# dherrera1911/sqfa

Measured on AMD Instinct MI355X. Metric: SPD pairwise-distance loss+grad evals/sec, higher is better.
Workload: dtype f32; 1 GPU; c3: C=1000 classes, n_dim=784, n_filters=16, smsqfa (m=16), 499500 unordered pairs per eval, inputs resident in HBM; parallelism=pair-tile shard over 1 GPU(s) + 1 all-reduce of [loss,flags,grad] per eval

## Files before the change

### include/sqfa_hip.h

```cpp
#ifndef SQFA_HIP_H
#define SQFA_HIP_H

#include <stddef.h>

#ifdef __cplusplus
extern "C" {
#endif

#define SQFA_F32 0
#define SQFA_F64 1

#define SQFA_OK                 0
#define SQFA_ERR_BAD_ARGUMENT  -1
#define SQFA_ERR_UNSUPPORTED_M -2
#define SQFA_ERR_WORKSPACE     -3
#define SQFA_ERR_LAUNCH        -4

int sqfa_hip_version(void);
const char *sqfa_hip_arch(void);
int sqfa_hip_max_dim(void);

const char *sqfa_hip_last_error(void);

int sqfa_airm_tiling(int nA, int nB, int m, int dtype,
                     int *tile_i, int *tile_j, int *n_tiles_i, int *n_tiles_j, int *padded_m);

size_t sqfa_airm_workspace_bytes(int nA, int nB, int m, int dtype);
size_t sqfa_airm_workspace_bytes_sharded(int nA, int nB, int m, int dtype, int shard_count, int geometry_policy);

typedef struct sqfa_airm_options {
  int geometry_policy;
  int class_factor_policy;
  unsigned long long *sweep_counter;
  int mean_metric_policy;
} sqfa_airm_options;

int sqfa_airm_pairwise(const void *A, int nA, const void *B, int nB, int m, int dtype,
                       double scale, double eps, int sqrt_mode,
                       const void *pair_weights, double uniform_weight,
                       int shard_index, int shard_count,
                       void *loss_out, void *gradA_out, void *gradB_out,
                       void *dist_out, void *eig_out, int *nonfinite_out,
                       void *workspace, size_t workspace_bytes, void *stream);
int sqfa_airm_pairwise_opt(const void *A, int nA, const void *B, int nB, int m, int dtype,
                           double scale, double eps, int sqrt_mode,
                           const void *pair_weights, double uniform_weight,
                           int shard_index, int shard_count,
                           void *loss_out, void *gradA_out, void *gradB_out,
                           void *dist_out, void *eig_out, int *nonfinite_out,
                           void *workspace, size_t workspace_bytes, void *stream,
                           const sqfa_airm_options *options);

size_t sqfa_bw_workspace_bytes(int nA, int nB, int m, int dtype);
size_t sqfa_bw_workspace_bytes_sharded(int nA, int nB, int m, int dtype, int shard_count, int geometry_policy);
int sqfa_bw_pairwise(const void *A, int nA, const void *B, int nB, int m, int dtype,
                     double eps, int sqrt_mode,
                     const void *pair_weights, double uniform_weight,
                     int shard_index, int shard_count,
                     void *loss_out, void *gradA_out, void *gradB_out,
                     void *dist_out, int *nonfinite_out,
                     void *workspace, size_t workspace_bytes, void *stream,
                     const sqfa_airm_options *options);

int sqfa_airm_eigenvalues_backward(const void *A, int nA, const void *B, int nB, int m, int dtype,
                                   const void *eig_weights, void *gradA_out, void *gradB_out,
                                   void *workspace, size_t workspace_bytes, void *stream,
                                   const sqfa_airm_options *options);

int sqfa_project_scatters(const void *F, int K, int D, const void *Psi, int C, int dtype, void *T_out,
                          void *stream);

size_t sqfa_packed_scatter_elems(int D);
int sqfa_pack_scatters(const void *Psi, int C, int D, int dtype, void *packed_out, void *stream);
int sqfa_project_scatters_packed(const void *F, int K, int D, const void *packed, int C, int dtype, void *T_out,
                                 void *stream);

int sqfa_feature_scatters(const void *F, int K, int D, const void *T, int C, int dtype, void *S_out, void *stream);
int sqfa_feature_scatters_backward(const void *G, const void *T, int C, int D, int K, int dtype, int n_groups,
                                   void *partial_out, void *stream);

int sqfa_feature_scatters_ex(const void *F, int K, int D, const void *T, int C, int dtype, double noise,
                             const void *means_f, void *S_out, void *stream);
int sqfa_feature_scatters_backward_ex(const void *G, int ldg, const void *T, int C, int D, int K, int dtype,
                                      int n_groups, int g_symmetric, void *partial_out, void *stream);
int sqfa_embed_backward_means(const void *gE, const void *means_f, int C, int K, int dtype, void *gm_out, void *stream);
int sqfa_sphere_forward(const void *X, int K, int D, int dtype, void *F_out, void *norms_out, void *stream);
int sqfa_sphere_backward(const void *X, const void *norms, int K, int D, int dtype, const void *partials, int n_groups,
                         const void *extra, const void *gloss, void *grad_out, void *stream);

int sqfa_lbfgs_max_history(void);
size_t sqfa_lbfgs_work_elems(int h, int n);
int sqfa_lbfgs_push(void *S, void *Y, void *SY, int h, int n, int slot, const void *s, const void *y, void *work,
                    int dtype, void *stream);
int sqfa_lbfgs_step_stats(const void *g, const void *g_prev, const void *d, double t, int n, void *y_out, void *s_out,
                          void *scalars_out, void *work, int dtype, void *stream);
int sqfa_lbfgs_direction(const void *S, const void *Y, const void *SY, int h, int n, const int *slots, int k,
                         const void *g, const void *H_diag, void *d_out, void *work, int dtype, void *stream);

int sqfa_gauss_pair_terms(const void *muA, const void *covA, int nA, const void *muB, const void *covB, int nB,
                          int m, int dtype, const void *gQ, const void *gLD, void *Q_out, void *LD_out,
                          void *gmuA_out, void *gcovA_out, void *stream);

#define SQFA_GAUSS_BHATTACHARYYA  0
#define SQFA_GAUSS_HELLINGER      1
// ... 26 lines not shown
```

### sqfa_amd/_lib.py

```python
import ctypes
import os

_HERE = os.path.dirname(os.path.abspath(__file__))
LIB_PATH = os.environ.get("SQFA_HIP_LIBRARY") or os.path.join(_HERE, "lib", "libsqfa_hip.so")

SQFA_F32, SQFA_F64 = 0, 1
SQFA_GAUSS_BHATTACHARYYA, SQFA_GAUSS_HELLINGER, SQFA_GAUSS_MAHALANOBIS_SQ, SQFA_GAUSS_MAHALANOBIS = 0, 1, 2, 3
SQFA_OK = 0
STATUS_TEXT = {
    -1: "bad argument",
    -2: "matrix size not supported by the native kernels",
    -3: "workspace too small",
    -4: "HIP launch failed",
}

class AirmOptions(ctypes.Structure):
    _fields_ = [("geometry_policy", ctypes.c_int), ("class_factor_policy", ctypes.c_int),
                ("sweep_counter", ctypes.c_void_p), ("mean_metric_policy", ctypes.c_int)]


_PAIRWISE_ARGS = [ctypes.c_void_p, ctypes.c_int, ctypes.c_void_p, ctypes.c_int, ctypes.c_int, ctypes.c_int,
                  ctypes.c_double, ctypes.c_double, ctypes.c_int,
                  ctypes.c_void_p, ctypes.c_double,
                  ctypes.c_int, ctypes.c_int,
                  ctypes.c_void_p, ctypes.c_void_p, ctypes.c_void_p,
                  ctypes.c_void_p, ctypes.c_void_p, ctypes.c_void_p,
                  ctypes.c_void_p, ctypes.c_size_t, ctypes.c_void_p]

_c_int_p = ctypes.POINTER(ctypes.c_int)
PROTOTYPES = {
    "sqfa_hip_version": (ctypes.c_int, []),
    "sqfa_hip_arch": (ctypes.c_char_p, []),
    "sqfa_hip_max_dim": (ctypes.c_int, []),
    "sqfa_hip_last_error": (ctypes.c_char_p, []),
    "sqfa_airm_tiling": (ctypes.c_int, [ctypes.c_int] * 4 + [_c_int_p] * 5),
    "sqfa_airm_workspace_bytes": (ctypes.c_size_t, [ctypes.c_int] * 4),
    "sqfa_airm_workspace_bytes_sharded": (ctypes.c_size_t, [ctypes.c_int] * 6),
    "sqfa_airm_pairwise": (ctypes.c_int, list(_PAIRWISE_ARGS)),
    "sqfa_airm_pairwise_opt": (ctypes.c_int, list(_PAIRWISE_ARGS) + [ctypes.POINTER(AirmOptions)]),
    "sqfa_bw_workspace_bytes": (ctypes.c_size_t, [ctypes.c_int] * 4),
    "sqfa_bw_workspace_bytes_sharded": (ctypes.c_size_t, [ctypes.c_int] * 6),
    "sqfa_bw_pairwise": (
        ctypes.c_int,
        [ctypes.c_void_p, ctypes.c_int, ctypes.c_void_p, ctypes.c_int, ctypes.c_int, ctypes.c_int,
         ctypes.c_double, ctypes.c_int, ctypes.c_void_p, ctypes.c_double, ctypes.c_int, ctypes.c_int,
         ctypes.c_void_p, ctypes.c_void_p, ctypes.c_void_p, ctypes.c_void_p, ctypes.c_void_p,
         ctypes.c_void_p, ctypes.c_size_t, ctypes.c_void_p, ctypes.POINTER(AirmOptions)],
    ),
    "sqfa_airm_eigenvalues_backward": (
        ctypes.c_int,
        [ctypes.c_void_p, ctypes.c_int, ctypes.c_void_p, ctypes.c_int, ctypes.c_int, ctypes.c_int,
         ctypes.c_void_p, ctypes.c_void_p, ctypes.c_void_p, ctypes.c_void_p, ctypes.c_size_t, ctypes.c_void_p,
         ctypes.POINTER(AirmOptions)],
    ),
    "sqfa_gauss_pair_terms": (
        ctypes.c_int,
        [ctypes.c_void_p, ctypes.c_void_p, ctypes.c_int, ctypes.c_void_p, ctypes.c_void_p, ctypes.c_int,
         ctypes.c_int, ctypes.c_int, ctypes.c_void_p, ctypes.c_void_p, ctypes.c_void_p, ctypes.c_void_p,
         ctypes.c_void_p, ctypes.c_void_p, ctypes.c_void_p],
    ),
    "sqfa_gauss_pairwise_workspace_bytes": (ctypes.c_size_t, [ctypes.c_int] * 3),
    "sqfa_gauss_pairwise_loss": (
        ctypes.c_int,
        [ctypes.c_void_p, ctypes.c_void_p, ctypes.c_int, ctypes.c_int, ctypes.c_int, ctypes.c_int,
         ctypes.c_double, ctypes.c_double, ctypes.c_void_p, ctypes.c_void_p, ctypes.c_void_p, ctypes.c_void_p,
         ctypes.c_void_p, ctypes.c_void_p, ctypes.c_size_t, ctypes.c_void_p],
    ),
    "sqfa_project_scatters": (
        ctypes.c_int,
        [ctypes.c_void_p, ctypes.c_int, ctypes.c_int, ctypes.c_void_p, ctypes.c_int, ctypes.c_int,
         ctypes.c_void_p, ctypes.c_void_p],
    ),
    "sqfa_packed_scatter_elems": (ctypes.c_size_t, [ctypes.c_int]),
    "sqfa_pack_scatters": (
        ctypes.c_int,
        [ctypes.c_void_p, ctypes.c_int, ctypes.c_int, ctypes.c_int, ctypes.c_void_p, ctypes.c_void_p],
    ),
    "sqfa_project_scatters_packed": (
        ctypes.c_int,
        [ctypes.c_void_p, ctypes.c_int, ctypes.c_int, ctypes.c_void_p, ctypes.c_int, ctypes.c_int,
         ctypes.c_void_p, ctypes.c_void_p],
    ),
    "sqfa_feature_scatters": (
        ctypes.c_int,
        [ctypes.c_void_p, ctypes.c_int, ctypes.c_int, ctypes.c_void_p, ctypes.c_int, ctypes.c_int,
         ctypes.c_void_p, ctypes.c_void_p],
    ),
    "sqfa_feature_scatters_backward": (
        ctypes.c_int,
        [ctypes.c_void_p, ctypes.c_void_p, ctypes.c_int, ctypes.c_int, ctypes.c_int, ctypes.c_int, ctypes.c_int,
         ctypes.c_void_p, ctypes.c_void_p],
    ),
# ... 89 lines not shown
```

### sqfa_amd/csrc/pair_inst.hip

```cpp
#include <type_traits>

#include "configs.hpp"
#include "pair_kernel.hpp"

#define SQFA_CAT_(a, b, c) a##b##_##c
#define SQFA_CAT(a, b, c) SQFA_CAT_(a, b, c)

#if defined(SQFA_RS) && SQFA_RS != 0
#include "pair_kernel_2d.hpp"
#define SQFA_ROW2D_MATCHES(T, MR, GC, CPL, TJ, WV, RS) \
  || (std::is_same<T, SQFA_T>::value && MR == SQFA_MR && GC == SQFA_G && CPL == SQFA_CPL && TJ == SQFA_TJ && WV == SQFA_WAVES && RS == SQFA_RS)
static_assert(false SQFA_CONFIGS2D_F32(SQFA_ROW2D_MATCHES) SQFA_CONFIGS2D_F64(SQFA_ROW2D_MATCHES),
              "Makefile CONFIGS2D and configs.hpp disagree");
namespace sqfa {
hipError_t SQFA_CAT(launch_pair2d_, SQFA_TAG, SQFA_MR)(const PairParams& p, hipStream_t stream) {
  return launch_pair_tiles_2d<PairCfg2D<SQFA_T, SQFA_MR, SQFA_G, SQFA_CPL, SQFA_TJ, SQFA_WAVES, SQFA_RS>>(p, stream);
}
hipError_t SQFA_CAT(launch_pair2d_bw_, SQFA_TAG, SQFA_MR)(const PairParams& p, hipStream_t stream) {
  return launch_pair_tiles_2d_bw<PairCfg2D<SQFA_T, SQFA_MR, SQFA_G, SQFA_CPL, SQFA_TJ, SQFA_WAVES, SQFA_RS>>(p, stream);
}
hipError_t SQFA_CAT(launch_factor2d_, SQFA_TAG, SQFA_MR)(const PairParams& p, hipStream_t stream) {
  return launch_class_factors<PairCfg2D<SQFA_T, SQFA_MR, SQFA_G, SQFA_CPL, SQFA_TJ, SQFA_WAVES, SQFA_RS>>(p, stream);
}
hipError_t SQFA_CAT(launch_classeig2d_, SQFA_TAG, SQFA_MR)(const void* LT, int n, int m, double* U, double* lam, hipStream_t stream) {
  return launch_class_eig<PairCfg2D<SQFA_T, SQFA_MR, SQFA_G, SQFA_CPL, SQFA_TJ, SQFA_WAVES, SQFA_RS>>(LT, n, m, U, lam, stream);
}
}
#else
#define SQFA_ROW_MATCHES(T, MR, G, CPL, TJ, WV) \
  || (std::is_same<T, SQFA_T>::value && MR == SQFA_MR && G == SQFA_G && CPL == SQFA_CPL && TJ == SQFA_TJ && WV == SQFA_WAVES)
static_assert(false SQFA_CONFIGS_F32(SQFA_ROW_MATCHES) SQFA_CONFIGS_F64(SQFA_ROW_MATCHES) SQFA_CONFIGS_F32_SMALL(SQFA_ROW_MATCHES)
              SQFA_CONFIGS_F64_SMALL(SQFA_ROW_MATCHES),
              "Makefile CONFIGS / CONFIGS_SMALL and configs.hpp disagree");
namespace sqfa {
hipError_t SQFA_CAT(launch_pair_, SQFA_TAG, SQFA_MR)(const PairParams& p, hipStream_t stream) {
  return launch_pair_tiles<PairCfg<SQFA_T, SQFA_MR, SQFA_G, SQFA_CPL, SQFA_TJ, SQFA_WAVES>>(p, stream);
}
hipError_t SQFA_CAT(launch_pair_bw_, SQFA_TAG, SQFA_MR)(const PairParams& p, hipStream_t stream) {
  return launch_pair_tiles_bw<PairCfg<SQFA_T, SQFA_MR, SQFA_G, SQFA_CPL, SQFA_TJ, SQFA_WAVES>>(p, stream);
}
hipError_t SQFA_CAT(launch_factor_, SQFA_TAG, SQFA_MR)(const PairParams& p, hipStream_t stream) {
  return launch_class_factors<PairCfg<SQFA_T, SQFA_MR, SQFA_G, SQFA_CPL, SQFA_TJ, SQFA_WAVES>>(p, stream);
}
hipError_t SQFA_CAT(launch_classeig_, SQFA_TAG, SQFA_MR)(const void* LT, int n, int m, double* U, double* lam, hipStream_t stream) {
  return launch_class_eig<PairCfg<SQFA_T, SQFA_MR, SQFA_G, SQFA_CPL, SQFA_TJ, SQFA_WAVES>>(LT, n, m, U, lam, stream);
}
}
#endif
```

### sqfa_amd/csrc/pair_kernel.hpp

```cpp
#pragma once
#include <hip/hip_runtime.h>
#include <stdint.h>

namespace sqfa {

struct PairParams {
  const void* LT;
  const void* Linv;
  const void* W;
  const void* EW;
  void* slab_grad;
  void* slab_loss;
  int* slab_flag;
  int* row_start;
  void* dist_out;
  void* eig_out;
  unsigned long long* sweep_counter;
  int nA, nB, m;
  int self_mode, sqrt_mode, want_grad;
  int shard_index, shard_count;
  int nbi, nbj;
  int tj;
  int factor_mode;
  const double* mean_linv;
// ... 1567 lines not shown
  class_jacobi_sweeps<T, MR, G, CPL>(x, D, 40);
  if (cls < n) {
#pragma unroll
    for (int c = 0; c < CPL; ++c) {
      const int col = c * G + g;
      if (col < m) {
        T a = T(0);
#pragma unroll
        for (int r = 0; r < MR; ++r) a = R::fma_(x[c][r], x[c][r], a);
        const T l = a * D[c];
        lam[(size_t)cls * m + col] = l;
        const T inv = R::sqrt_(D[c]) / R::sqrt_(l);
#pragma unroll
        for (int r = 0; r < MR; ++r) {
          if (r < m) U[((size_t)cls * m + r) * m + col] = x[c][r] * inv;
        }
      }
    }
  }
}

template <typename Cfg>
hipError_t launch_class_eig(const void* LT, int n, int m, double* U, double* lam, hipStream_t stream) {
  using T = typename Cfg::type;
  using FC = FactorCfg<T, Cfg::MR>;
  const int blocks = (n + FC::PPW - 1) / FC::PPW;
  hipLaunchKernelGGL((class_eig_kernel<FC>), dim3(blocks), dim3(64), 0, stream, static_cast<const T*>(LT), n, m, U, lam);
  return hipGetLastError();
}

template <typename Cfg>
hipError_t launch_class_factors(const PairParams& p, hipStream_t stream) {
  if constexpr (!Cfg::DENSE_FACTOR) {
    return hipSuccess;
  } else {
    using T = typename Cfg::type;
    using FC = FactorCfg<T, Cfg::MR>;
    const long pairs = p.self_mode ? (long)p.nA * (p.nA - 1) / 2 : (long)p.nA * p.nB;
    if (p.factor_mode < 0 || (p.factor_mode == 0 && pairs / p.shard_count < Cfg::FACTOR_MIN_PAIRS)) return hipSuccess;
    const int blocks = (p.nA + FC::PPW - 1) / FC::PPW;
    if constexpr (Cfg::MEAN_METRIC) {
      if (p.mean_linv != nullptr) {
        hipLaunchKernelGGL((class_factor_mean_kernel<FC>), dim3(blocks), dim3(64), 0, stream,
                           static_cast<T*>(const_cast<void*>(p.LT)), p.nA, Cfg::FACTOR_SWEEPS, p.mean_linv);
        return hipGetLastError();
      }
    }
    hipLaunchKernelGGL((class_factor_kernel<FC>), dim3(blocks), dim3(64), 0, stream,
                       static_cast<T*>(const_cast<void*>(p.LT)), p.nA, Cfg::FACTOR_SWEEPS);
    return hipGetLastError();
  }
}

}
```

### sqfa_amd/csrc/sqfa_api.hip

```cpp
#include <hip/hip_runtime.h>
#include <stdio.h>
#include <string.h>

#include <algorithm>
#include <atomic>
#include <mutex>
#include <utility>
#include <vector>

#include "../../include/sqfa_hip.h"
#include "configs.hpp"
#include "pair_kernel.hpp"
#include "pair_kernel_2d.hpp"
#include "pair_kernel_lds.hpp"

namespace sqfa {

#define SQFA_DECL_F32(T, MR, G, CPL, TJ, WV) \
  hipError_t launch_pair_f32_##MR(const PairParams&, hipStream_t);   \
  hipError_t launch_pair_bw_f32_##MR(const PairParams&, hipStream_t); \
  hipError_t launch_factor_f32_##MR(const PairParams&, hipStream_t); \
  hipError_t launch_classeig_f32_##MR(const void*, int, int, double*, double*, hipStream_t);
#define SQFA_DECL_F64(T, MR, G, CPL, TJ, WV) \
  hipError_t launch_pair_f64_##MR(const PairParams&, hipStream_t);   \
  hipError_t launch_pair_bw_f64_##MR(const PairParams&, hipStream_t); \
  hipError_t launch_factor_f64_##MR(const PairParams&, hipStream_t); \
  hipError_t launch_classeig_f64_##MR(const void*, int, int, double*, double*, hipStream_t);
SQFA_CONFIGS_F32(SQFA_DECL_F32)
SQFA_CONFIGS_F64(SQFA_DECL_F64)
#define SQFA_DECL_F32S(T, MR, G, CPL, TJ, WV) \
  hipError_t launch_pair_f32s_##MR(const PairParams&, hipStream_t);  \
  hipError_t launch_pair_bw_f32s_##MR(const PairParams&, hipStream_t); \
  hipError_t launch_factor_f32s_##MR(const PairParams&, hipStream_t);
SQFA_CONFIGS_F32_SMALL(SQFA_DECL_F32S)
#define SQFA_DECL_F64S(T, MR, G, CPL, TJ, WV) \
  hipError_t launch_pair_f64s_##MR(const PairParams&, hipStream_t);  \
  hipError_t launch_pair_bw_f64s_##MR(const PairParams&, hipStream_t); \
  hipError_t launch_factor_f64s_##MR(const PairParams&, hipStream_t);
SQFA_CONFIGS_F64_SMALL(SQFA_DECL_F64S)

#define SQFA_DECL2D_F32(T, MR, GC, CPL, TJ, WV, RS) \
  hipError_t launch_pair2d_f32_##MR(const PairParams&, hipStream_t); \
  hipError_t launch_pair2d_bw_f32_##MR(const PairParams&, hipStream_t); \
  hipError_t launch_factor2d_f32_##MR(const PairParams&, hipStream_t); \
  hipError_t launch_classeig2d_f32_##MR(const void*, int, int, double*, double*, hipStream_t);
#define SQFA_DECL2D_F64(T, MR, GC, CPL, TJ, WV, RS) \
  hipError_t launch_pair2d_f64_##MR(const PairParams&, hipStream_t); \
  hipError_t launch_pair2d_bw_f64_##MR(const PairParams&, hipStream_t); \
  hipError_t launch_factor2d_f64_##MR(const PairParams&, hipStream_t); \
  hipError_t launch_classeig2d_f64_##MR(const void*, int, int, double*, double*, hipStream_t);
SQFA_CONFIGS2D_F32(SQFA_DECL2D_F32)
SQFA_CONFIGS2D_F64(SQFA_DECL2D_F64)

struct Geometry {
  int dtype, MR, TJ, TI, WV;
  hipError_t (*launch)(const PairParams&, hipStream_t);
  hipError_t (*factor)(const PairParams&, hipStream_t);
  hipError_t (*eig)(const void*, int, int, double*, double*, hipStream_t);
  hipError_t (*launch_bw)(const PairParams&, hipStream_t);
  bool mean_metric;
  long factor_min_pairs;
};
template <typename Cfg>
static Geometry make_geometry(decltype(Geometry::launch) launch, decltype(Geometry::factor) factor, decltype(Geometry::eig) eig,
                              decltype(Geometry::launch_bw) launch_bw) {
  return Geometry{sizeof(typename Cfg::type) == 4 ? SQFA_F32 : SQFA_F64, Cfg::MR, Cfg::TJ, Cfg::TI, Cfg::WAVES, launch, factor, eig,
                  launch_bw, Cfg::MEAN_METRIC, Cfg::FACTOR_MIN_PAIRS};
}

static bool find_geometry(int m, int dtype, long pairs, Geometry* out, int geometry_mode = 0) {
  bool found = false;
  Geometry best{};
  auto consider = [&](const Geometry& g) {
    if (g.dtype == dtype && m <= g.MR && (!found || g.MR < best.MR)) {
      best = g;
      found = true;
    }
  };
  auto consider_small = [&](Geometry g, long max_pairs) {
    g.eig = best.eig;
    if (g.dtype == dtype && g.MR == best.MR && (geometry_mode > 0 || pairs < max_pairs)) best = g;
  };
#define SQFA_ROW_F32(T, MR, G, CPL, TJ, WV) \
  consider(make_geometry<PairCfg<T, MR, G, CPL, TJ, WV>>(launch_pair_f32_##MR, launch_factor_f32_##MR, launch_classeig_f32_##MR, launch_pair_bw_f32_##MR));
#define SQFA_ROW_F64(T, MR, G, CPL, TJ, WV) \
  consider(make_geometry<PairCfg<T, MR, G, CPL, TJ, WV>>(launch_pair_f64_##MR, launch_factor_f64_##MR, launch_classeig_f64_##MR, launch_pair_bw_f64_##MR));
#define SQFA_ROW2D_F32(T, MR, GC, CPL, TJ, WV, RS) \
  consider(make_geometry<PairCfg2D<T, MR, GC, CPL, TJ, WV, RS>>(launch_pair2d_f32_##MR, launch_factor2d_f32_##MR, launch_classeig2d_f32_##MR, launch_pair2d_bw_f32_##MR));
#define SQFA_ROW2D_F64(T, MR, GC, CPL, TJ, WV, RS) \
  consider(make_geometry<PairCfg2D<T, MR, GC, CPL, TJ, WV, RS>>(launch_pair2d_f64_##MR, launch_factor2d_f64_##MR, launch_classeig2d_f64_##MR, launch_pair2d_bw_f64_##MR));
#define SQFA_ROW_F32S(T, MR, G, CPL, TJ, WV) \
  consider_small(make_geometry<PairCfg<T, MR, G, CPL, TJ, WV>>(launch_pair_f32s_##MR, launch_factor_f32s_##MR, nullptr, launch_pair_bw_f32s_##MR), small_launch_max_pairs(MR));
#define SQFA_ROW_F64S(T, MR, G, CPL, TJ, WV) \
  consider_small(make_geometry<PairCfg<T, MR, G, CPL, TJ, WV>>(launch_pair_f64s_##MR, launch_factor_f64s_##MR, nullptr, launch_pair_bw_f64s_##MR), small_launch_max_pairs_f64(MR));
  SQFA_CONFIGS_F32(SQFA_ROW_F32)
  SQFA_CONFIGS_F64(SQFA_ROW_F64)
  SQFA_CONFIGS2D_F32(SQFA_ROW2D_F32)
  SQFA_CONFIGS2D_F64(SQFA_ROW2D_F64)
  if (found && geometry_mode >= 0 && pairs >= 0) {
    SQFA_CONFIGS_F32_SMALL(SQFA_ROW_F32S)
    SQFA_CONFIGS_F64_SMALL(SQFA_ROW_F64S)
  }
  if (found) *out = best;
  return found;
}
static long pair_count(int nA, int nB, int shard_count) {
  const long p = nB == 0 ? (long)nA * (nA - 1) / 2 : (long)nA * nB;
  return p / (shard_count > 0 ? shard_count : 1);
}

constexpr int kSpdMaxDim = kRegMaxDim;

static thread_local char g_last_error[256] = "";

struct EventPair { hipEvent_t a, b; };
static std::atomic<bool> g_profile{false};
static std::vector<EventPair> g_events;
static std::mutex g_events_mutex;
}
bool sqfa_profile_enabled() { return sqfa::g_profile.load(); }
std::vector<std::pair<hipEvent_t, hipEvent_t>>& sqfa_project_events() {
  static std::vector<std::pair<hipEvent_t, hipEvent_t>> ev;
  return ev;
}
std::mutex& sqfa_project_events_mutex() {
  static std::mutex m;
  return m;
}
namespace sqfa {

static size_t align_up(size_t v) { return (v + 255) & ~(size_t)255; }

struct WorkspaceLayout {
  size_t off_lt, off_linv, off_slab, off_loss, off_flag, off_rows, off_mean, total;
};
constexpr int kMeanParts = 32;

static long shard_tiles(int nA, int nBeff, int TI, int tj, int self_mode, int shard_index, int shard_count) {
  const int nbi = (nA + TI - 1) / TI, nbj = (nBeff + tj - 1) / tj;
// ... 76 lines not shown
  WorkspaceLayout w;
  size_t owned = 0;
  for (int r = 0; r < pl.shard_count; ++r)
    owned = std::max(owned, (size_t)shard_tiles(pl.nA, pl.nBeff, pl.TI, pl.tj, pl.self_mode, r, pl.shard_count));
  const size_t tri = (size_t)pl.MR * (pl.MR + 1) / 2;
  size_t o = 0;
  w.off_lt = o;   o = align_up(o + (size_t)pl.nA * pl.MR * pl.MR * pl.esz);
  w.off_linv = o; o = align_up(o + (size_t)pl.nBeff * tri * pl.esz);
  w.off_slab = o; o = align_up(o + owned * (size_t)(pl.TI + pl.tj) * tri * pl.esz);
  w.off_loss = o; o = align_up(o + owned * pl.esz);
  w.off_flag = o; o = align_up(o + owned * 2 * sizeof(int));
  w.off_rows = o; o = align_up(o + ((size_t)pl.nbi + 1) * sizeof(int));
  w.off_mean = o;
  w.total = o;
  return w;
}

constexpr long kLdsMinTiles = 1024;

static bool make_plan(int nA, int nB, int m, int dtype, int shard_count, int geometry_mode, PairPlan* out,
                      bool any_width = false) {
  PairPlan pl{};
  pl.nA = nA;
  pl.m = m;
  pl.dtype = dtype;
  pl.shard_count = shard_count;
  pl.self_mode = nB == 0 ? 1 : 0;
  pl.nBeff = nB == 0 ? nA : nB;
  pl.esz = dtype == SQFA_F32 ? 4 : 8;
  pl.lds = m > kRegMaxDim;
  if (pl.lds) {
    if (m > kLdsMaxDim) return false;
    pl.MR = lds_padded_size(m);
    pl.TI = pl.TJ = 16;
    while (pl.TI * pl.TJ > 4 && shard_tiles(nA, pl.nBeff, pl.TI, pl.TJ, pl.self_mode, 0, 1) < kLdsMinTiles) {
      if (pl.TJ >= pl.TI) pl.TJ /= 2;
      else pl.TI /= 2;
    }
    pl.tj = pl.TJ;
  } else {
    if (!find_geometry(m, dtype, pair_count(nA, nB, shard_count), &pl.g, geometry_mode)) return false;
    pl.MR = pl.g.MR;
    pl.TI = pl.g.TI;
    pl.TJ = pl.g.TJ;
    pl.tj = choose_tile_width(nA, pl.nBeff, pl.g, pl.self_mode, shard_count);
  }
  pl.nbi = (nA + pl.TI - 1) / pl.TI;
  pl.nbj = (pl.nBeff + pl.tj - 1) / pl.tj;
  pl.w = pl.lds ? layout_lds(pl) : layout(pl, any_width);
  *out = pl;
  return true;
}

__device__ __forceinline__ double fast_rsqrt(double x) {
  double y = __builtin_amdgcn_rsq(x);
  y = y * (1.5 - 0.5 * x * y * y);
  y = y * (1.5 - 0.5 * x * y * y);
  return y;
}

template <typename T>
__global__ __launch_bounds__(256) void mean_partial_kernel(const T* __restrict__ S, int n, int m, double* __restrict__ out) {
  const int b = blockIdx.x, P = gridDim.x;
  for (int e = threadIdx.x; e < m * m; e += 256) {
    double a0 = 0.0, a1 = 0.0;
    int c = b;
    for (; c + P < n; c += 2 * P) {
      a0 += (double)S[(size_t)c * m * m + e];
      a1 += (double)S[(size_t)(c + P) * m * m + e];
    }
    if (c < n) a0 += (double)S[(size_t)c * m * m + e];
    out[(size_t)b * m * m + e] = a0 + a1;
  }
}

template <typename T, int MAXM>
__global__ __launch_bounds__(256) void cholesky_kernel(const T* __restrict__ S, int m, int MR,
                                                       T* __restrict__ LT, T* __restrict__ Linv,
                                                       int* __restrict__ row_start, PairParams pp, int TI,
                                                       int n_classes = 0, const double* __restrict__ mean_parts = nullptr,
                                                       int n_parts = 0, double* __restrict__ mean_linv = nullptr) {
  if (row_start != nullptr && blockIdx.x == 0) write_row_start_table(pp, TI, row_start);
  __shared__ double a[MAXM][MAXM + 1];
  __shared__ double b[MAXM][MAXM + 1];
  __shared__ double rd[MAXM];
  const int c = blockIdx.x, t = threadIdx.x;
  const bool mean_block = mean_parts != nullptr && c == n_classes;
  if (mean_block) {
    const double inv_n = 1.0 / (double)n_classes;
    for (int idx = t; idx < m * m; idx += 256) {
      double acc = 0.0;
      for (int q = 0; q < n_parts; ++q) acc += mean_parts[(size_t)q * m * m + idx];
      a[idx / m][idx % m] = acc * inv_n;
      b[idx / m][idx % m] = 0.0;
    }
  } else {
    const T* s = S + (size_t)c * m * m;
    for (int idx = t; idx < m * m; idx += 256) {
      a[idx / m][idx % m] = (double)s[idx];
      b[idx / m][idx % m] = 0.0;
    }
  }
  __syncthreads();
  for (int k = 0; k < m; ++k) {
    const double akk = a[k][k];
    double rk = __builtin_amdgcn_rcp(akk);
    rk = rk * (2.0 - akk * rk);
    rk = rk * (2.0 - akk * rk);
    if (!(akk > 0.0)) rk = __builtin_nan("");
    const int n = m - k - 1;
    for (int e = t; e < n * n; e += 256) {
      const int r = k + 1 + e / n, c2 = k + 1 + e % n;
// ... 574 lines not shown
    (void)hipEventDestroy(ev.a);
    (void)hipEventDestroy(ev.b);
  }
  g_events.clear();
  if (tile_kernel_ms_total) *tile_kernel_ms_total = total;
  if (launches) *launches = n;
  return SQFA_OK;
}

int sqfa_project_profile_read(double* kernel_ms_total, int* launches) {
  double total = 0.0;
  int n = 0;
  std::lock_guard<std::mutex> lock(sqfa_project_events_mutex());
  for (auto& ev : sqfa_project_events()) {
    float ms = 0.f;
    if (hipEventSynchronize(ev.second) == hipSuccess && hipEventElapsedTime(&ms, ev.first, ev.second) == hipSuccess) {
      total += ms;
      ++n;
    }
    (void)hipEventDestroy(ev.first);
    (void)hipEventDestroy(ev.second);
  }
  sqfa_project_events().clear();
  if (kernel_ms_total) *kernel_ms_total = total;
  if (launches) *launches = n;
  return SQFA_OK;
}

int sqfa_airm_tiling(int nA, int nB, int m, int dtype, int* tile_i, int* tile_j, int* n_tiles_i,
                     int* n_tiles_j, int* padded_m) {
  if (nA < 1 || nB < 0 || m < 1 || !known_dtype(dtype)) return SQFA_ERR_BAD_ARGUMENT;
  PairPlan pl;
  if (!make_plan(nA, nB, m, dtype, 1, 0, &pl)) return SQFA_ERR_UNSUPPORTED_M;
  if (tile_i) *tile_i = pl.TI;
  if (tile_j) *tile_j = pl.TJ;
  if (n_tiles_i) *n_tiles_i = pl.nbi;
  if (n_tiles_j) *n_tiles_j = (pl.nBeff + pl.TJ - 1) / pl.TJ;
  if (padded_m) *padded_m = pl.MR;
  return SQFA_OK;
}

size_t sqfa_airm_workspace_bytes(int nA, int nB, int m, int dtype) {
  if (nA < 1 || nB < 0 || m < 1 || !known_dtype(dtype)) return 0;
  PairPlan regular, small;
  if (!make_plan(nA, nB, m, dtype, 1, -1, &regular, true) || !make_plan(nA, nB, m, dtype, 1, 1, &small, true)) return 0;
  return std::max(regular.w.total, small.w.total);
}

static int pairwise_impl(const void* A, int nA, const void* B, int nB, int m, int dtype, double scale,
                         double eps, int sqrt_mode, const void* pair_weights, double uniform_weight,
                         int shard_index, int shard_count, void* loss_out, void* gradA_out,
                         void* gradB_out, void* dist_out, void* eig_out, int* nonfinite_out,
                         void* workspace, size_t workspace_bytes, void* stream_, const void* eig_weights,
                         const sqfa_airm_options* options) {
  hipStream_t stream = static_cast<hipStream_t>(stream_);
  const int rc = validate_pair_call(A, nA, B, nB, m, dtype, shard_index, shard_count, workspace);
  if (rc != SQFA_OK) return rc;
  PairPlan pl;
  if (!make_plan(nA, nB, m, dtype, shard_count, options ? clamp_policy(options->geometry_policy) : 0, &pl))
    return fail(SQFA_ERR_UNSUPPORTED_M, "matrix size not supported", hipSuccess);
  if (workspace_bytes < pl.w.total) return fail(SQFA_ERR_WORKSPACE, "workspace too small", hipSuccess);
  char* ws = static_cast<char*>(workspace);
  PairParams p = make_pair_params(pl, ws, shard_index, scale, eps, sqrt_mode, pair_weights, uniform_weight, gradA_out != nullptr,
                                  dist_out, options);
  p.EW = eig_weights;
  p.eig_out = eig_out;

  const int mean_mode = options ? clamp_policy(options->mean_metric_policy) : 0;
  const bool want_mean = pl.g.mean_metric && mean_mode > 0 && p.factor_mode >= 0 &&
                         (p.factor_mode > 0 || pair_count(nA, nB, shard_count) >= pl.g.factor_min_pairs) && nA >= 2;
  double* mean_parts = reinterpret_cast<double*>(ws + pl.w.off_mean);
  double* mean_linv = mean_parts + (size_t)kMeanParts * pl.MR * pl.MR;
  const int n_parts = nA < kMeanParts ? nA : kMeanParts;
  if (want_mean) {
    if (dtype == SQFA_F32) hipLaunchKernelGGL(mean_partial_kernel<float>, dim3(n_parts), dim3(256), 0, stream, static_cast<const float*>(A), nA, m, mean_parts);
    else hipLaunchKernelGGL(mean_partial_kernel<double>, dim3(n_parts), dim3(256), 0, stream, static_cast<const double*>(A), nA, m, mean_parts);
    p.mean_linv = mean_linv;
  }
  hipError_t e = launch_factors(pl, p, stream, A, nA, ws + pl.w.off_lt, pl.self_mode ? ws + pl.w.off_linv : nullptr, p.row_start,
                                want_mean ? mean_parts : nullptr, n_parts, mean_linv);
  if (!pl.self_mode && e == hipSuccess) e = launch_factors(pl, p, stream, B, nB, nullptr, ws + pl.w.off_linv, nullptr);
  if (e != hipSuccess) return fail(SQFA_ERR_LAUNCH, pl.lds ? "cholesky_lds_kernel" : "cholesky_kernel", e);
  if (pl.g.factor != nullptr) {
    e = pl.g.factor(p, stream);
    if (e != hipSuccess) return fail(SQFA_ERR_LAUNCH, "class_factor_kernel", e);
  }

  e = launch_profiled(stream, [&] { return pl.lds ? launch_pair_lds(dtype == SQFA_F64, p, pl.TI, pl.MR, stream) : pl.g.launch(p, stream); });
  if (e != hipSuccess) return fail(SQFA_ERR_LAUNCH, pl.lds ? "pair_lds_kernel" : "pair_tile_kernel", e);

  e = launch_finalize(pl, p, gradA_out, gradB_out, loss_out, nonfinite_out, stream);
  if (e != hipSuccess) return fail(SQFA_ERR_LAUNCH, "finalize_kernel", e);
  return SQFA_OK;
}

struct BwExtra {
  size_t off_tr, off_h, off_hsum, off_sinv, off_g, off_w, total;
};
static void bw_tiles(int nA, int nB, int m, int dtype, int* nbi, int* TJ) {
  PairPlan regular, small;
  make_plan(nA, nB, m, dtype, 1, -1, &regular);
  make_plan(nA, nB, m, dtype, 1, 1, &small);
  *nbi = std::max(regular.nbi, small.nbi);
  *TJ = std::max(regular.TJ, small.TJ);
}
static BwExtra bw_extra(size_t base, int nA, int nB, int m, int dtype) {
  const int nBeff = nB == 0 ? nA : nB;
  int nbi, TJ;
  bw_tiles(nA, nB, m, dtype, &nbi, &TJ);
  BwExtra x;
  size_t o = base;
  x.off_tr = o;   o = align_up(o + (size_t)(nA + nBeff) * sizeof(double));
  x.off_h = o;    o = align_up(o + (size_t)nbi * (nBeff + TJ) * sizeof(double));
  x.off_hsum = o; o = align_up(o + (size_t)nBeff * sizeof(double));
  x.off_sinv = o; o = align_up(o + (size_t)nBeff * m * m * sizeof(double));
  x.off_g = o;    o = align_up(o + (size_t)nBeff * m * m * sizeof(double));
  x.off_w = o;    o = align_up(o + (size_t)nBeff * m * m * sizeof(double));
  x.total = o;
  return x;
}

static int bw_impl(const void* A, int nA, const void* B, int nB, int m, int dtype, double eps, int sqrt_mode,
                   const void* pair_weights, double uniform_weight, int shard_index, int shard_count, void* loss_out,
                   void* gradA_out, void* gradB_out, void* dist_out, int* nonfinite_out, void* workspace,
                   size_t workspace_bytes, void* stream_, const sqfa_airm_options* options) {
  hipStream_t stream = static_cast<hipStream_t>(stream_);
  const int rc = validate_pair_call(A, nA, B, nB, m, dtype, shard_index, shard_count, workspace);
  if (rc != SQFA_OK) return rc;
  PairPlan pl;
  if (!make_plan(nA, nB, m, dtype, shard_count, options ? clamp_policy(options->geometry_policy) : 0, &pl))
    return fail(SQFA_ERR_UNSUPPORTED_M, "matrix size not supported", hipSuccess);
  const BwExtra x = bw_extra(pl.w.total, nA, nB, m, dtype);
  if (workspace_bytes < x.total) return fail(SQFA_ERR_WORKSPACE, "workspace too small", hipSuccess);
  char* ws = static_cast<char*>(workspace);
  double* tr = reinterpret_cast<double*>(ws + x.off_tr);
  double* sinv = reinterpret_cast<double*>(ws + x.off_sinv);
// ... 32 lines not shown
  e = launch_profiled(stream, [&] { return pl.lds ? launch_pair_lds_bw(dtype == SQFA_F64, p, pl.TI, pl.MR, stream) : pl.g.launch_bw(p, stream); });
  if (e != hipSuccess) return fail(SQFA_ERR_LAUNCH, "pair_tile_kernel (Bures-Wasserstein)", e);

  PairParams q = p;
  q.want_grad = 0;
  e = launch_finalize(pl, q, nullptr, nullptr, loss_out, nonfinite_out, stream);
  if (e != hipSuccess) return fail(SQFA_ERR_LAUNCH, "finalize_kernel", e);
  if (p.want_grad) {
    double* G = reinterpret_cast<double*>(ws + x.off_g);
    double* W = reinterpret_cast<double*>(ws + x.off_w);
    double* hs = reinterpret_cast<double*>(ws + x.off_hsum);
    void* outB = pl.self_mode ? gradA_out : gradB_out;
    e = by_dtype([&](auto zero) {
      using T = decltype(zero);
      hipLaunchKernelGGL(finalize_bw_kernel<T>, dim3((nA + pl.nBeff) * finalize_bw_bpc(pl.MR * (pl.MR + 1) / 2)), dim3(256), 0, stream,
                         p, pl.TI, pl.tj, pl.MR, static_cast<T*>(gradA_out), G, hs);
      if (outB != nullptr)
        hipLaunchKernelGGL(bw_sandwich_kernel<T>, dim3(pl.nBeff), dim3(256), 0, stream, m, sinv, G, W, hs, static_cast<T*>(outB),
                           pl.self_mode);
    });
    if (e != hipSuccess) return fail(SQFA_ERR_LAUNCH, "finalize_bw_kernel", e);
  }
  return SQFA_OK;
}

size_t sqfa_airm_workspace_bytes_sharded(int nA, int nB, int m, int dtype, int shard_count, int geometry_policy) {
  PairPlan pl;
  if (shard_count < 1 || nA < 1 || nB < 0 || m < 1 || !known_dtype(dtype) ||
      !make_plan(nA, nB, m, dtype, shard_count, clamp_policy(geometry_policy), &pl))
    return 0;
  return pl.w.total;
}

int sqfa_airm_pairwise(const void* A, int nA, const void* B, int nB, int m, int dtype, double scale,
                       double eps, int sqrt_mode, const void* pair_weights, double uniform_weight,
                       int shard_index, int shard_count, void* loss_out, void* gradA_out,
                       void* gradB_out, void* dist_out, void* eig_out, int* nonfinite_out,
                       void* workspace, size_t workspace_bytes, void* stream_) {
  return pairwise_impl(A, nA, B, nB, m, dtype, scale, eps, sqrt_mode, pair_weights, uniform_weight, shard_index,
                       shard_count, loss_out, gradA_out, gradB_out, dist_out, eig_out, nonfinite_out, workspace,
                       workspace_bytes, stream_, nullptr, nullptr);
}

int sqfa_airm_pairwise_opt(const void* A, int nA, const void* B, int nB, int m, int dtype, double scale,
                           double eps, int sqrt_mode, const void* pair_weights, double uniform_weight,
                           int shard_index, int shard_count, void* loss_out, void* gradA_out,
                           void* gradB_out, void* dist_out, void* eig_out, int* nonfinite_out,
                           void* workspace, size_t workspace_bytes, void* stream_, const sqfa_airm_options* options) {
  return pairwise_impl(A, nA, B, nB, m, dtype, scale, eps, sqrt_mode, pair_weights, uniform_weight, shard_index,
                       shard_count, loss_out, gradA_out, gradB_out, dist_out, eig_out, nonfinite_out, workspace,
                       workspace_bytes, stream_, nullptr, options);
}

int sqfa_airm_eigenvalues_backward(const void* A, int nA, const void* B, int nB, int m, int dtype,
                                   const void* eig_weights, void* gradA_out, void* gradB_out,
                                   void* workspace, size_t workspace_bytes, void* stream_,
                                   const sqfa_airm_options* options) {
  if (eig_weights == nullptr || gradA_out == nullptr) {
    g_last_error[0] = 0;
    return fail(SQFA_ERR_BAD_ARGUMENT, "eig_weights / gradA_out", hipSuccess);
  }
  return pairwise_impl(A, nA, B, nB, m, dtype, 1.0, 0.0, 0, nullptr, 0.0, 0, 1, nullptr, gradA_out, gradB_out,
                       nullptr, nullptr, nullptr, workspace, workspace_bytes, stream_, eig_weights, options);
}

size_t sqfa_bw_workspace_bytes(int nA, int nB, int m, int dtype) {
  const size_t base = sqfa_airm_workspace_bytes(nA, nB, m, dtype);
  return base == 0 ? 0 : bw_extra(align_up(base), nA, nB, m, dtype).total;
}

size_t sqfa_bw_workspace_bytes_sharded(int nA, int nB, int m, int dtype, int shard_count, int geometry_policy) {
  const size_t base = sqfa_airm_workspace_bytes_sharded(nA, nB, m, dtype, shard_count, geometry_policy);
  return base == 0 ? 0 : bw_extra(align_up(base), nA, nB, m, dtype).total;
}

int sqfa_bw_pairwise(const void* A, int nA, const void* B, int nB, int m, int dtype, double eps, int sqrt_mode,
                     const void* pair_weights, double uniform_weight, int shard_index, int shard_count, void* loss_out,
                     void* gradA_out, void* gradB_out, void* dist_out, int* nonfinite_out, void* workspace,
                     size_t workspace_bytes, void* stream_, const sqfa_airm_options* options) {
  return bw_impl(A, nA, B, nB, m, dtype, eps, sqrt_mode, pair_weights, uniform_weight, shard_index, shard_count, loss_out,
                 gradA_out, gradB_out, dist_out, nonfinite_out, workspace, workspace_bytes, stream_, options);
}

size_t sqfa_spd_function_workspace_bytes(int n, int m, int dtype) {
  Geometry g;
  if (n < 1 || m < 1 || !known_dtype(dtype) || !find_geometry(m, dtype, -1, &g, -1)) return 0;
  return align_up((size_t)n * g.MR * g.MR * (dtype == SQFA_F32 ? 4 : 8));
}

int sqfa_spd_function(const void* S, int n, int m, int dtype, int kind, void* F_out, double* U_out, double* lam_out,
                      void* workspace, size_t workspace_bytes, void* stream_) {
  hipStream_t stream = static_cast<hipStream_t>(stream_);
  g_last_error[0] = 0;
  if (S == nullptr || n < 1 || m < 1 || U_out == nullptr || lam_out == nullptr || workspace == nullptr)
    return fail(SQFA_ERR_BAD_ARGUMENT, "null/size argument", hipSuccess);
  if (dtype != SQFA_F32 && dtype != SQFA_F64) return fail(SQFA_ERR_BAD_ARGUMENT, "dtype", hipSuccess);
  if (kind != SQFA_SPD_LOG && kind != SQFA_SPD_SQRT && kind != SQFA_SPD_INV_SQRT) return fail(SQFA_ERR_BAD_ARGUMENT, "kind", hipSuccess);
  Geometry g;
  if (!find_geometry(m, dtype, -1, &g, -1) || g.eig == nullptr) return fail(SQFA_ERR_UNSUPPORTED_M, "matrix size not supported", hipSuccess);
  if (workspace_bytes < sqfa_spd_function_workspace_bytes(n, m, dtype)) return fail(SQFA_ERR_WORKSPACE, "workspace too small", hipSuccess);
  PairParams p;
  memset(&p, 0, sizeof(p));
  launch_cholesky(dtype, m, stream, S, n, g.MR, workspace, nullptr, nullptr, p, g.TI);
  hipError_t e = hipGetLastError();
  if (e != hipSuccess) return fail(SQFA_ERR_LAUNCH, "cholesky_kernel", e);
  e = g.eig(workspace, n, m, U_out, lam_out, stream);
// ... 35 lines not shown
```

Baseline: 1379 evals/s.

## Fuse class Cholesky, triangular inverse and Jacobi factor into one prologue kernel

```diff
diff --git a/include/sqfa_hip.h b/include/sqfa_hip.h
--- a/include/sqfa_hip.h
+++ b/include/sqfa_hip.h
@@ -50,6 +50,14 @@
                            void *dist_out, void *eig_out, int *nonfinite_out,
                            void *workspace, size_t workspace_bytes, void *stream,
                            const sqfa_airm_options *options);
+int sqfa_airm_pairwise_prologue(const void *A, int nA, const void *B, int nB, int m, int dtype,
+                                double scale, double eps, int sqrt_mode,
+                                const void *pair_weights, double uniform_weight,
+                                int shard_index, int shard_count,
+                                void *loss_out, void *gradA_out, void *gradB_out,
+                                void *dist_out, void *eig_out, int *nonfinite_out,
+                                void *workspace, size_t workspace_bytes, void *stream,
+                                const sqfa_airm_options *options, int prologue_policy);
 
 size_t sqfa_bw_workspace_bytes(int nA, int nB, int m, int dtype);
 size_t sqfa_bw_workspace_bytes_sharded(int nA, int nB, int m, int dtype, int shard_count, int geometry_policy);
diff --git a/sqfa_amd/_lib.py b/sqfa_amd/_lib.py
--- a/sqfa_amd/_lib.py
+++ b/sqfa_amd/_lib.py
@@ -38,6 +38,7 @@
     "sqfa_airm_workspace_bytes_sharded": (ctypes.c_size_t, [ctypes.c_int] * 6),
     "sqfa_airm_pairwise": (ctypes.c_int, list(_PAIRWISE_ARGS)),
     "sqfa_airm_pairwise_opt": (ctypes.c_int, list(_PAIRWISE_ARGS) + [ctypes.POINTER(AirmOptions)]),
+    "sqfa_airm_pairwise_prologue": (ctypes.c_int, list(_PAIRWISE_ARGS) + [ctypes.POINTER(AirmOptions), ctypes.c_int]),
     "sqfa_bw_workspace_bytes": (ctypes.c_size_t, [ctypes.c_int] * 4),
     "sqfa_bw_workspace_bytes_sharded": (ctypes.c_size_t, [ctypes.c_int] * 6),
     "sqfa_bw_pairwise": (
diff --git a/sqfa_amd/csrc/pair_inst.hip b/sqfa_amd/csrc/pair_inst.hip
--- a/sqfa_amd/csrc/pair_inst.hip
+++ b/sqfa_amd/csrc/pair_inst.hip
@@ -42,6 +42,10 @@
 hipError_t SQFA_CAT(launch_factor_, SQFA_TAG, SQFA_MR)(const PairParams& p, hipStream_t stream) {
   return launch_class_factors<PairCfg<SQFA_T, SQFA_MR, SQFA_G, SQFA_CPL, SQFA_TJ, SQFA_WAVES>>(p, stream);
 }
+hipError_t SQFA_CAT(launch_prologue_, SQFA_TAG, SQFA_MR)(const PairParams& p, hipStream_t stream, const void* S, void* LT, void* Linv,
+                                                         int TI) {
+  return launch_class_prologue<PairCfg<SQFA_T, SQFA_MR, SQFA_G, SQFA_CPL, SQFA_TJ, SQFA_WAVES>>(p, stream, S, LT, Linv, TI);
+}
 hipError_t SQFA_CAT(launch_classeig_, SQFA_TAG, SQFA_MR)(const void* LT, int n, int m, double* U, double* lam, hipStream_t stream) {
   return launch_class_eig<PairCfg<SQFA_T, SQFA_MR, SQFA_G, SQFA_CPL, SQFA_TJ, SQFA_WAVES>>(LT, n, m, U, lam, stream);
 }
diff --git a/sqfa_amd/csrc/pair_kernel.hpp b/sqfa_amd/csrc/pair_kernel.hpp
--- a/sqfa_amd/csrc/pair_kernel.hpp
+++ b/sqfa_amd/csrc/pair_kernel.hpp
@@ -1643,4 +1643,186 @@
   }
 }
 
-}
+__device__ __forceinline__ double fast_rsqrt(double x) {
+  double y = __builtin_amdgcn_rsq(x);
+  y = y * (1.5 - 0.5 * x * y * y);
+  y = y * (1.5 - 0.5 * x * y * y);
+  return y;
+}
+
+template <typename Cfg>
+constexpr bool fused_prologue_cfg() {
+  return Cfg::DENSE_FACTOR && Cfg::MR >= 12 && Cfg::MR <= 20 && FactorCfg<typename Cfg::type, Cfg::MR>::G == 16;
+}
+
+template <typename Cfg>
+__global__ __launch_bounds__(64 * Cfg::PPW) void class_prologue_kernel(const typename Cfg::io_type* __restrict__ S, int m, int n,
+                                                                        typename Cfg::io_type* __restrict__ LT,
+                                                                        typename Cfg::io_type* __restrict__ Linv,
+                                                                        int* __restrict__ row_start, PairParams pp, int TI,
+                                                                        int max_sweeps) {
+  using Tio = typename Cfg::io_type;
+#if SQFA_FACTOR_F64
+  using T = double;
+#else
+  using T = Tio;
+#endif
+  using R = Real<T>;
+  constexpr int MR = Cfg::MR, G = Cfg::G, CPL = Cfg::CPL, PPW = Cfg::PPW;
+  constexpr int P = MR + 1, TRI = MR * (MR + 1) / 2, NS = (TRI + 63) / 64;
+  static_assert(64 * PPW == 256, "write_row_start_table needs 256 threads");
+  static_assert(MR < 32, "unpacked inverse factors only");
+  if (row_start != nullptr && blockIdx.x == 0) write_row_start_table(pp, TI, row_start);
+  __shared__ double s_a[PPW][MR * P];
+  __shared__ double s_b[PPW][MR * P];
+  __shared__ double s_rd[PPW][MR];
+  const int wave = threadIdx.x >> 6, lane = threadIdx.x & 63;
+  const int cls_w = blockIdx.x * PPW + wave;
+  const bool live = cls_w < n;
+  const int cls = live ? cls_w : n - 1;
+  double* a = s_a[wave];
+  double* b = s_b[wave];
+  double* rd = s_rd[wave];
+  auto wave_sync = [] {
+    __builtin_amdgcn_fence(__ATOMIC_ACQ_REL, "wavefront");
+    __builtin_amdgcn_wave_barrier();
+  };
+  const Tio* s = S + (size_t)cls * m * m;
+  double v[NS];
+  int er[NS], ec[NS];
+  bool on[NS];
+#pragma unroll
+  for (int q = 0; q < NS; ++q) {
+    const int e = q * 64 + lane;
+    int r = (int)((__fsqrt_rn(8.0f * (float)e + 1.0f) - 1.0f) * 0.5f);
+    while ((r + 1) * (r + 2) / 2 <= e) ++r;
+    while (r * (r + 1) / 2 > e) --r;
+    on[q] = e < TRI && r < m;
+    er[q] = on[q] ? r : 0;
+    ec[q] = on[q] ? e - r * (r + 1) / 2 : 0;
+    v[q] = on[q] ? (double)s[er[q] * m + ec[q]] : 0.0;
+    if (on[q]) a[er[q] * P + ec[q]] = v[q];
+  }
+  wave_sync();
+  for (int k = 0; k < m; ++k) {
+    const double akk = a[k * P + k];
+    double rk = __builtin_amdgcn_rcp(akk);
+    rk = rk * (2.0 - akk * rk);
+    rk = rk * (2.0 - akk * rk);
+    if (!(akk > 0.0)) rk = __builtin_nan("");
+    double xr[NS], xc[NS];
+#pragma unroll
+    for (int q = 0; q < NS; ++q) {
+      xr[q] = a[er[q] * P + k];
+      xc[q] = a[ec[q] * P + k];
+    }
+#pragma unroll
+    for (int q = 0; q < NS; ++q) {
+      const double nv = v[q] - xr[q] * xc[q] * rk;
+      if (on[q] && ec[q] > k) {
+        v[q] = nv;
+        a[er[q] * P + ec[q]] = nv;
+      }
+    }
+    wave_sync();
+  }
+  if (lane < m) rd[lane] = fast_rsqrt(a[lane * P + lane]);
+  wave_sync();
+#pragma unroll
+  for (int q = 0; q < NS; ++q) {
+    if (on[q]) a[er[q] * P + ec[q]] = v[q] * rd[ec[q]];
+  }
+  wave_sync();
+  {
+    constexpr int NJ = (MR + 3) / 4;
+    const int part = lane & 3;
+    for (int r = 0; r < m; ++r) {
+      for (int cb = 0; cb <= r; cb += 16) {
+        const int col = cb + (lane >> 2);
+        double av[NJ], bv[NJ];
+#pragma unroll
+        for (int j = 0; j < NJ; ++j) {
+          const int k = col + part + 4 * j;
+          const bool ok = k < r;
+          av[j] = a[r * P + (ok ? k : 0)];
+          bv[j] = b[ok ? k * P + col : 0];
+        }
+        double acc = 0.0;
+#pragma unroll
+        for (int j = 0; j < NJ; ++j) {
+          if (col + part + 4 * j < r) acc += av[j] * bv[j];
+        }
+        acc += __shfl_xor(acc, 1, 64);
+        acc += __shfl_xor(acc, 2, 64);
+        if (part == 0 && col <= r) b[r * P + col] = ((col == r ? 1.0 : 0.0) - acc) * rd[r];
+      }
+      wave_sync();
+    }
+  }
+  const size_t base = (size_t)cls * MR * MR;
+  auto lt_value = [&](const double* img, int col, int k) -> double {
+    return (col < m && k < m) ? (k >= col ? img[k * P + col] : 0.0) : (col == k ? 1.0 : 0.0);
+  };
+  if (Linv != nullptr && live) {
+    for (int idx = lane; idx < MR * MR; idx += 64) {
+      const int r = idx / MR, k = idx % MR;
+      const double val = (r < m && k < m) ? (k <= r ? b[r * P + k] : 0.0) : (r == k ? 1.0 : 0.0);
+      Linv[base + idx] = (Tio)val;
+    }
+  }
+  if (LT == nullptr) return;
+  if (max_sweeps <= 0) {
+    if (live) {
+      for (int idx = lane; idx < MR * MR; idx += 64) LT[base + idx] = (Tio)lt_value(a, idx / MR, idx % MR);
+    }
+    return;
+  }
+  __syncthreads();
+  if (wave != 0) return;
+  const int g = lane % G, grp = lane / G;
+  const int cls_g = blockIdx.x * PPW + grp;
+  const double* img = s_a[grp];
+  T x[CPL][MR];
+#pragma unroll
+  for (int c = 0; c < CPL; ++c) {
+    const int col = c * G + g;
+    const bool real_col = col < MR;
+#pragma unroll
+    for (int k = 0; k < MR; ++k) x[c][k] = real_col ? (T)(Tio)lt_value(img, col, k) : T(0);
+  }
+  T D[CPL];
+#pragma unroll
+  for (int c = 0; c < CPL; ++c) D[c] = T(1);
+  class_jacobi_sweeps<T, MR, G, CPL>(x, D, max_sweeps);
+  if (cls_g < n) {
+    Tio* lt = LT + (size_t)cls_g * (MR * MR);
+#pragma unroll
+    for (int c = 0; c < CPL; ++c) {
+      const int col = c * G + g;
+      if (col < MR) {
+        const T dc = R::sqrt_(D[c]);
+        Tio* dst = lt + (size_t)col * MR;
+#pragma unroll
+        for (int r = 0; r < MR; ++r) dst[r] = (Tio)(x[c][r] * dc);
+      }
+    }
+  }
+}
+
+template <typename Cfg>
+hipError_t launch_class_prologue(const PairParams& p, hipStream_t stream, const void* S, void* LT, void* Linv, int TI) {
+  if constexpr (!fused_prologue_cfg<Cfg>()) {
+    return hipErrorInvalidConfiguration;
+  } else {
+    using T = typename Cfg::type;
+    using FC = FactorCfg<T, Cfg::MR>;
+    const long pairs = p.self_mode ? (long)p.nA * (p.nA - 1) / 2 : (long)p.nA * p.nB;
+    const bool skip = p.factor_mode < 0 || (p.factor_mode == 0 && pairs / p.shard_count < Cfg::FACTOR_MIN_PAIRS);
+    const int blocks = (p.nA + FC::PPW - 1) / FC::PPW;
+    hipLaunchKernelGGL((class_prologue_kernel<FC>), dim3(blocks), dim3(64 * FC::PPW), 0, stream, static_cast<const T*>(S), p.m, p.nA,
+                       static_cast<T*>(LT), static_cast<T*>(Linv), p.row_start, p, TI, skip ? 0 : Cfg::FACTOR_SWEEPS);
+    return hipGetLastError();
+  }
+}
+
+}
diff --git a/sqfa_amd/csrc/sqfa_api.hip b/sqfa_amd/csrc/sqfa_api.hip
--- a/sqfa_amd/csrc/sqfa_api.hip
+++ b/sqfa_amd/csrc/sqfa_api.hip
@@ -20,11 +20,13 @@
   hipError_t launch_pair_f32_##MR(const PairParams&, hipStream_t);   \
   hipError_t launch_pair_bw_f32_##MR(const PairParams&, hipStream_t); \
   hipError_t launch_factor_f32_##MR(const PairParams&, hipStream_t); \
+  hipError_t launch_prologue_f32_##MR(const PairParams&, hipStream_t, const void*, void*, void*, int); \
   hipError_t launch_classeig_f32_##MR(const void*, int, int, double*, double*, hipStream_t);
 #define SQFA_DECL_F64(T, MR, G, CPL, TJ, WV) \
   hipError_t launch_pair_f64_##MR(const PairParams&, hipStream_t);   \
   hipError_t launch_pair_bw_f64_##MR(const PairParams&, hipStream_t); \
   hipError_t launch_factor_f64_##MR(const PairParams&, hipStream_t); \
+  hipError_t launch_prologue_f64_##MR(const PairParams&, hipStream_t, const void*, void*, void*, int); \
   hipError_t launch_classeig_f64_##MR(const void*, int, int, double*, double*, hipStream_t);
 SQFA_CONFIGS_F32(SQFA_DECL_F32)
 SQFA_CONFIGS_F64(SQFA_DECL_F64)
@@ -58,14 +60,15 @@
   hipError_t (*factor)(const PairParams&, hipStream_t);
   hipError_t (*eig)(const void*, int, int, double*, double*, hipStream_t);
   hipError_t (*launch_bw)(const PairParams&, hipStream_t);
+  hipError_t (*prologue)(const PairParams&, hipStream_t, const void* S, void* LT, void* Linv, int TI);
   bool mean_metric;
   long factor_min_pairs;
 };
 template <typename Cfg>
 static Geometry make_geometry(decltype(Geometry::launch) launch, decltype(Geometry::factor) factor, decltype(Geometry::eig) eig,
-                              decltype(Geometry::launch_bw) launch_bw) {
+                              decltype(Geometry::launch_bw) launch_bw, decltype(Geometry::prologue) prologue = nullptr) {
   return Geometry{sizeof(typename Cfg::type) == 4 ? SQFA_F32 : SQFA_F64, Cfg::MR, Cfg::TJ, Cfg::TI, Cfg::WAVES, launch, factor, eig,
-                  launch_bw, Cfg::MEAN_METRIC, Cfg::FACTOR_MIN_PAIRS};
+                  launch_bw, fused_prologue_cfg<Cfg>() ? prologue : nullptr, Cfg::MEAN_METRIC, Cfg::FACTOR_MIN_PAIRS};
 }
 
 static bool find_geometry(int m, int dtype, long pairs, Geometry* out, int geometry_mode = 0) {
@@ -79,12 +82,13 @@
   };
   auto consider_small = [&](Geometry g, long max_pairs) {
     g.eig = best.eig;
+    g.prologue = best.prologue;
     if (g.dtype == dtype && g.MR == best.MR && (geometry_mode > 0 || pairs < max_pairs)) best = g;
   };
 #define SQFA_ROW_F32(T, MR, G, CPL, TJ, WV) \
-  consider(make_geometry<PairCfg<T, MR, G, CPL, TJ, WV>>(launch_pair_f32_##MR, launch_factor_f32_##MR, launch_classeig_f32_##MR, launch_pair_bw_f32_##MR));
+  consider(make_geometry<PairCfg<T, MR, G, CPL, TJ, WV>>(launch_pair_f32_##MR, launch_factor_f32_##MR, launch_classeig_f32_##MR, launch_pair_bw_f32_##MR, launch_prologue_f32_##MR));
 #define SQFA_ROW_F64(T, MR, G, CPL, TJ, WV) \
-  consider(make_geometry<PairCfg<T, MR, G, CPL, TJ, WV>>(launch_pair_f64_##MR, launch_factor_f64_##MR, launch_classeig_f64_##MR, launch_pair_bw_f64_##MR));
+  consider(make_geometry<PairCfg<T, MR, G, CPL, TJ, WV>>(launch_pair_f64_##MR, launch_factor_f64_##MR, launch_classeig_f64_##MR, launch_pair_bw_f64_##MR, launch_prologue_f64_##MR));
 #define SQFA_ROW2D_F32(T, MR, GC, CPL, TJ, WV, RS) \
   consider(make_geometry<PairCfg2D<T, MR, GC, CPL, TJ, WV, RS>>(launch_pair2d_f32_##MR, launch_factor2d_f32_##MR, launch_classeig2d_f32_##MR, launch_pair2d_bw_f32_##MR));
 #define SQFA_ROW2D_F64(T, MR, GC, CPL, TJ, WV, RS) \
@@ -267,12 +271,6 @@
   return true;
 }
 
-__device__ __forceinline__ double fast_rsqrt(double x) {
-  double y = __builtin_amdgcn_rsq(x);
-  y = y * (1.5 - 0.5 * x * y * y);
-  y = y * (1.5 - 0.5 * x * y * y);
-  return y;
-}
 
 template <typename T>
 __global__ __launch_bounds__(256) void mean_partial_kernel(const T* __restrict__ S, int n, int m, double* __restrict__ out) {
@@ -953,7 +951,7 @@
                          int shard_index, int shard_count, void* loss_out, void* gradA_out,
                          void* gradB_out, void* dist_out, void* eig_out, int* nonfinite_out,
                          void* workspace, size_t workspace_bytes, void* stream_, const void* eig_weights,
-                         const sqfa_airm_options* options) {
+                         const sqfa_airm_options* options, int prologue_policy = 0) {
   hipStream_t stream = static_cast<hipStream_t>(stream_);
   const int rc = validate_pair_call(A, nA, B, nB, m, dtype, shard_index, shard_count, workspace);
   if (rc != SQFA_OK) return rc;
@@ -978,11 +976,15 @@
     else hipLaunchKernelGGL(mean_partial_kernel<double>, dim3(n_parts), dim3(256), 0, stream, static_cast<const double*>(A), nA, m, mean_parts);
     p.mean_linv = mean_linv;
   }
-  hipError_t e = launch_factors(pl, p, stream, A, nA, ws + pl.w.off_lt, pl.self_mode ? ws + pl.w.off_linv : nullptr, p.row_start,
-                                want_mean ? mean_parts : nullptr, n_parts, mean_linv);
+  const bool fused = !pl.lds && pl.g.prologue != nullptr && !want_mean && prologue_policy >= 0;
+  void* linvA = pl.self_mode ? ws + pl.w.off_linv : nullptr;
+  hipError_t e = fused ? pl.g.prologue(p, stream, A, ws + pl.w.off_lt, linvA, pl.TI)
+                       : launch_factors(pl, p, stream, A, nA, ws + pl.w.off_lt, linvA, p.row_start,
+                                        want_mean ? mean_parts : nullptr, n_parts, mean_linv);
+  if (fused && e != hipSuccess) return fail(SQFA_ERR_LAUNCH, "class_prologue_kernel", e);
   if (!pl.self_mode && e == hipSuccess) e = launch_factors(pl, p, stream, B, nB, nullptr, ws + pl.w.off_linv, nullptr);
   if (e != hipSuccess) return fail(SQFA_ERR_LAUNCH, pl.lds ? "cholesky_lds_kernel" : "cholesky_kernel", e);
-  if (pl.g.factor != nullptr) {
+  if (!fused && pl.g.factor != nullptr) {
     e = pl.g.factor(p, stream);
     if (e != hipSuccess) return fail(SQFA_ERR_LAUNCH, "class_factor_kernel", e);
   }
@@ -1121,6 +1123,17 @@
                        workspace_bytes, stream_, nullptr, options);
 }
 
+int sqfa_airm_pairwise_prologue(const void* A, int nA, const void* B, int nB, int m, int dtype, double scale,
+                                double eps, int sqrt_mode, const void* pair_weights, double uniform_weight,
+                                int shard_index, int shard_count, void* loss_out, void* gradA_out,
+                                void* gradB_out, void* dist_out, void* eig_out, int* nonfinite_out,
+                                void* workspace, size_t workspace_bytes, void* stream_, const sqfa_airm_options* options,
+                                int prologue_policy) {
+  return pairwise_impl(A, nA, B, nB, m, dtype, scale, eps, sqrt_mode, pair_weights, uniform_weight, shard_index,
+                       shard_count, loss_out, gradA_out, gradB_out, dist_out, eig_out, nonfinite_out, workspace,
+                       workspace_bytes, stream_, nullptr, options, prologue_policy);
+}
+
 int sqfa_airm_eigenvalues_backward(const void* A, int nA, const void* B, int nB, int m, int dtype,
                                    const void* eig_weights, void* gradA_out, void* gradB_out,
                                    void* workspace, size_t workspace_bytes, void* stream_,
```

Result: no change. 1374 evals/s (-0.3%).
